# chensh236/ComputerVisionImageStich2

Measured on AMD Instinct MI355X. Metric: warp+blend MPix/s at 4096x4096x3 f32, higher is better.
Workload: dtype f32 (f64 accumulators)

## Files before the change

computervisionimagestich2_amd/capi.py:

```python
import ctypes as C
import os
import re

import numpy as np

_HERE = os.path.dirname(os.path.abspath(__file__))
LIB_PATH = os.environ.get("STITCH_LIB", os.path.join(_HERE, "libstitch_hip.so"))

KERNELS = ("compose", "seam", "mask", "vv_x_fwd", "vv_x_bwd", "vv_y_fwd", "vv_y_bwd", "decimate", "collapse_top", "collapse",
           "collapse_l0", "vv_xbyf", "vv_x_fwd_src", "coarse")
KERNEL_SYMBOLS = {"compose": "k_src_index (source-fused) / k_compose", "seam": "k_seam", "mask": "k_mask", "vv_x_fwd": "k_vv_x_fwd<T, false, false>", "vv_x_bwd": "k_vv_x_bwd",
                  "vv_y_fwd": "k_vv_y_fwd1 / k_vv_y_fwd", "vv_y_bwd": "k_vv_y_bwd_dec", "decimate": "k_decimate", "collapse_top": "k_blend_top",
                  "collapse": "k_collapse<float, false>", "collapse_l0": "k_collapse<T, true>", "vv_xbyf": "k_vv_xbyf<false, float, 0, false>", "vv_x_fwd_src": "k_vv_x_fwd<T, true, false>",
                  "coarse": "k_coarse"}


class StitchError(RuntimeError):
    def __init__(self, code, text):
        super().__init__(f"stitch error {code}: {text}")
        self.code = code


OK, ERR_ARG, ERR_EMPTY_MIDROW, ERR_ZERO_OVERLAP, ERR_PYRAMID, ERR_HIP, ERR_NO_DEVICE = 0, -1, -2, -3, -4, -5, -6

# ... 73 lines not shown
    ("stitch_sift_expn_table", None, vp), ("stitch_sift_elem", None, f64, vp),
)

_lib = None


def lib():
    global _lib
    if _lib is None:
        if not os.path.exists(LIB_PATH):
            raise ImportError(f"{LIB_PATH} is missing: build it with `python -c 'import __graft_entry__ as g; g.build()'` "
                              "(make -C computervisionimagestich2_amd/csrc). There is no CPU fallback.")
        try:
            import torch
        except ImportError:
            pass
        L = C.CDLL(LIB_PATH)
        for name, (res, args) in SIGNATURES.items():
            try:
                f = getattr(L, name)
            except AttributeError:
                raise ImportError(f"{LIB_PATH} does not export {name}: it was built from another include/stitch.h") from None
            f.restype, f.argtypes = res, args
        _lib = L
    return _lib


def _chk(rc):
    if rc < 0:
        raise StitchError(rc, lib().stitch_last_error().decode())
    return rc


def _p(a):
    return a.ctypes.data_as(C.c_void_p)


def _fn(stem, a):
    sfx = {"uint8": "u8", "float32": "f32"}.get(str(a.dtype).rpartition(".")[2])
    if sfx is None:
        raise TypeError(f"unsupported pixel type {a.dtype}")
    return getattr(lib(), stem + sfx)


def _img(a):
    a = np.ascontiguousarray(a)
# ... 596 lines not shown
            assert tuple(out.shape) == (3, self.ch, self.cw) and out.dtype == frame.dtype == mosaic.dtype
            assert frame.dtype == items[0][0].dtype, "one pixel type per batch"
            fn = fn or _fn("stitch_dev_pairs_", frame)
            d.frame, d.fw, d.fh = frame.data_ptr(), frame.shape[2], frame.shape[1]
            d.p = _map8(p)
            d.offx, d.offy = float(offx), float(offy)
            d.mosaic, d.mw, d.mh = mosaic.data_ptr(), mosaic.shape[2], mosaic.shape[1]
            d.ox, d.oy, d.out = int(ox), int(oy), out.data_ptr()
            if out8 is not None:
                import torch
                assert out8.is_cuda and out8.is_contiguous() and out8.dtype == torch.uint8 and tuple(out8.shape) == (3, self.ch, self.cw)
                d.out_u8 = out8.data_ptr()
        _chk(fn(self._h, arr, len(items), _stream()))
        return [it[7] for it in items]

    def status(self, index=0):
        s = Seam()
        _chk(lib().stitch_plan_status_at(self._h, int(index), C.byref(s)))
        return s

    def clear_fault(self):
        _chk(lib().stitch_plan_clear_fault(self._h))

    def set_handoff_spin_limit(self, polls):
        _chk(lib().stitch_plan_set_handoff_spin_limit(self._h, int(polls)))

    def set_profiling_kernel(self, name):
        _chk(lib().stitch_plan_set_profiling_kernel(self._h, KERNELS.index(name)))

    def set_profiling(self, on):
        _chk(lib().stitch_plan_set_profiling(self._h, int(bool(on))))

    def read_profile(self):
        ms, n, l0 = (C.c_double * len(KERNELS))(), (C.c_int * len(KERNELS))(), (C.c_double * len(KERNELS))()
        _chk(lib().stitch_plan_read_profile(self._h, ms, n, l0))
        return {KERNELS[i]: (ms[i], n[i], l0[i]) for i in range(len(KERNELS))}


class Band(_Handle):
    _destroy = "stitch_band_destroy"

    def __init__(self, cw, ch, rank, nranks, split_levels, opts=None):
        self._h = C.c_void_p()
        _chk(lib().stitch_band_create(int(cw), int(ch), int(rank), int(nranks), int(split_levels), C.byref(_opts(opts)), C.byref(self._h)))
        self.cw, self.ch, self.rank, self.nranks, self.split_levels = int(cw), int(ch), int(rank), int(nranks), int(split_levels)
        tot = C.c_int()
# ... 53 lines not shown
```

computervisionimagestich2_amd/csrc/k_fused_sweep.inc:

```
typedef unsigned long long u64;
typedef __attribute__((address_space(1))) u64 gu64;
typedef __attribute__((address_space(1))) unsigned gu32;

struct Wavefront {
    u64* yg;
    int mask_l0;
    unsigned* counter;
    unsigned* abort;
    unsigned* sticky;
    int NR, NC, NP;
    unsigned epoch;
    unsigned spin_limit;
    ZeroTiles zt;
    int ph, y0;
    const double* resume;
    int early_read;
    unsigned long long* dbg;
};

#ifndef STITCH_XBYF_SLEEP
#define STITCH_XBYF_SLEEP 32
#endif
constexpr int WF_GRAN = 7;
__device__ __forceinline__ void granules_publish(u64* base, int lane, unsigned tag, double a, double b, double c, unsigned extra) {
    const u64 w[3] = {(u64)__double_as_longlong(a), (u64)__double_as_longlong(b), (u64)__double_as_longlong(c)};
    __hip_atomic_store((gu64*)(base + 6 * WAVE + lane), ((u64)tag << 32) | extra, __ATOMIC_RELAXED, __HIP_MEMORY_SCOPE_AGENT);
#pragma unroll
    for (int i = 0; i < 3; ++i) {
        __hip_atomic_store((gu64*)(base + (2 * i) * WAVE + lane), ((u64)tag << 32) | (w[i] & 0xffffffffu), __ATOMIC_RELAXED,
                           __HIP_MEMORY_SCOPE_AGENT);
        __hip_atomic_store((gu64*)(base + (2 * i + 1) * WAVE + lane), ((u64)tag << 32) | (w[i] >> 32), __ATOMIC_RELAXED,
                           __HIP_MEMORY_SCOPE_AGENT);
    }
}
__device__ __forceinline__ void granules_issue(const u64* base, int lane, u64 g[WF_GRAN]) {
#pragma unroll
    for (int i = 0; i < WF_GRAN; ++i) g[i] = __hip_atomic_load((gu64*)(base + i * WAVE + lane), __ATOMIC_RELAXED, __HIP_MEMORY_SCOPE_AGENT);
}
__device__ __forceinline__ bool granules_accept(const u64 g[WF_GRAN], unsigned tag, double& a, double& b, double& c, unsigned& extra) {
    bool ok = true;
#pragma unroll
    for (int i = 0; i < WF_GRAN; ++i) ok &= (unsigned)(g[i] >> 32) == tag;
    if (!__all(ok)) return false;
    extra = (unsigned)g[6];
    a = __longlong_as_double((long long)((g[0] & 0xffffffffu) | (g[1] << 32)));
    b = __longlong_as_double((long long)((g[2] & 0xffffffffu) | (g[3] << 32)));
    c = __longlong_as_double((long long)((g[4] & 0xffffffffu) | (g[5] << 32)));
    return true;
}
__device__ __forceinline__ bool granules_consume(const u64* base, int lane, unsigned tag, unsigned* abort, unsigned* sticky,
                                                 unsigned spin_limit, double& a, double& b, double& c, unsigned& extra, bool brisk = false) {
    for (unsigned spins = 0;; ++spins) {
        unsigned seen = 0;
        if (lane == 0)
            seen = (unsigned)(__hip_atomic_load((gu64*)(base + 5 * WAVE + (WAVE - 1)), __ATOMIC_RELAXED, __HIP_MEMORY_SCOPE_AGENT) >> 32);
        seen = __shfl(seen, 0, 64);
        if (seen == tag) {
            u64 g[WF_GRAN];
            bool ok = true;
#pragma unroll
            for (int i = 0; i < WF_GRAN; ++i) {
                g[i] = __hip_atomic_load((gu64*)(base + i * WAVE + lane), __ATOMIC_RELAXED, __HIP_MEMORY_SCOPE_AGENT);
                ok &= (unsigned)(g[i] >> 32) == tag;
            }
            if (__all(ok)) {
                extra = (unsigned)g[6];
                a = __longlong_as_double((long long)((g[0] & 0xffffffffu) | (g[1] << 32)));
                b = __longlong_as_double((long long)((g[2] & 0xffffffffu) | (g[3] << 32)));
                c = __longlong_as_double((long long)((g[4] & 0xffffffffu) | (g[5] << 32)));
                return true;
            }
        }
        {
            if ((spins & 31) == 31) {
                unsigned ab = 0;
                if (lane == 0) ab = __hip_atomic_load((gu32*)abort, __ATOMIC_RELAXED, __HIP_MEMORY_SCOPE_AGENT);
                ab = __shfl(ab, 0, 64);
                if (ab != 0 || spins > spin_limit) {
                    if (lane == 0) {
                        __hip_atomic_store((gu32*)abort, 1u, __ATOMIC_RELAXED, __HIP_MEMORY_SCOPE_AGENT);
                        atomicAdd(sticky, 1u);
                    }
                    return false;
                }
            }
            if (brisk)
                __builtin_amdgcn_s_sleep(2);
            else
                __builtin_amdgcn_s_sleep(STITCH_XBYF_SLEEP);
        }
    }
}

struct Recompute {
    const float* in;
    const double* ckpt;
    const SeamDev* seam;
    ZeroTiles zi;
};
template <bool STAMP, typename PX = float, int MODE = 0, bool BANDED = false>
__global__ __launch_bounds__(64) void k_vv_xbyf(float* __restrict__ data, int w, int h, int pitch, VVK k,
                                                 const double* __restrict__ state_x, long lines, double* __restrict__ state_y,
                                                 Wavefront wf, Recompute rc, typename CollapseSrc<PX, MODE == 2>::type pa) {
    __shared__ __attribute__((aligned(16))) float tile[TS * TP];
    const int lane = threadIdx.x;
    const unsigned nbands = (unsigned)wf.NP * wf.NR;
    unsigned long long seg[8] = {0, 0, 0, 0, 0, 0, 0, 0}, t0 = 0, t1 = 0;
    auto stamp = [&](int i) {
        if (STAMP) {
            t1 = __builtin_amdgcn_s_memtime();
            seg[i] += t1 - t0;
            t0 = t1;
        }
    };
    if (STAMP) t0 = __builtin_amdgcn_s_memtime();
    bool dead = false;
    while (!dead) {
        unsigned q = 0;
        if (lane == 0) q = atomicAdd(wf.counter, 1u);
        q = __builtin_amdgcn_readfirstlane(__shfl(q, 0, 64));
        if (q >= nbands) break;
        const int R = (int)(q / wf.NP), p = (int)(q % wf.NP);
        const int r0 = R * TS, nrows = min(TS, h - r0);
        const int ph = BANDED ? wf.ph : h, y0 = BANDED ? wf.y0 : 0;
// ... 52 lines not shown
#pragma unroll
                for (int i = 0; i < 16; ++i) pre[i] = v;
            } else if (MODE == 1)
                tile_load(in_base, pitch, C * TS, lane, pre);
            else if (gen_frame) {
                if (rc.zi.flags && rc.zi.flags[rc.zi.index(src_pr, R, C)]) {
                    const float o = __uint_as_float(off_outside<PX>());
#pragma unroll
                    for (int i = 0; i < 16; ++i) pre[i] = f4{o, o, o, o};
                } else
                    tile_load(idx_rows, pitch, C * TS, lane, pre);
            }
            if (MODE != 0 && !zero) fetch_ckpt(C);
            return zero;
        };
        auto gather_tile = [&](int C, bool zero) {
            if constexpr (MODE == 2) {
                if (zero || gen_mask) return;
                if (gen_mosaic) mosaic_indices<PX>(ms, C * TS, lane, r0, w, pre);
                src_gather<PX>(rs, pre, pre);
            }
        };
        bool next_zero = false, spec = true;
        if (!const_rows) {
            next_zero = fetch_tile(wf.NC - 1);
            gather_tile(wf.NC - 1, next_zero);
        }
        for (int C = wf.NC - 1; C >= 0; --C) {
            const int c0 = C * TS, ncols = min(TS, w - c0);
            const bool tile_zero = next_zero;
            u64* slot = wf.yg + ((size_t)p * wf.NC + C) * WF_GRAN * WAVE;
            u64 early[WF_GRAN];
            const bool early_on = R > 0 && wf.early_read && (spec || (C & 3) == 0);
            if (early_on) granules_issue(slot, lane, early);
            double f1 = n1, f2 = n2, f3 = n3;
            if (!const_rows) {
                if constexpr (MODE == 2)
                    if (!tile_zero && !gen_mask) src_finish<PX>(gen_frame, pre);
                tile_to_lds(tile, lane, pre);
                if (C > 0) next_zero = fetch_tile(C - 1);
            }
            __syncthreads();
            stamp(1);
            if (MODE != 0 && !const_rows && !tile_zero) {
                float* row = tile + lane * TP;
                if (C == 0) f1 = f2 = f3 = (double)row[0] / k.sumsq;
                const int jfull = ncols & ~15;
                for (int jb = 0; jb < jfull; jb += 16) {
                    float xs[16];
#pragma unroll
                    for (int qq = 0; qq < 4; ++qq) *reinterpret_cast<f4*>(xs + 4 * qq) = *reinterpret_cast<const f4*>(row + jb + 4 * qq);
#pragma unroll
                    for (int u = 0; u < 16; ++u) {
                        double v0 = (double)xs[u];
                        v0 += f1 * k.f1;
                        v0 += f2 * k.f2;
                        v0 += f3 * k.f3;
// ... 51 lines not shown
                        v0 += v3 * k.f3;
                        xs[u] = (float)v0;
                        v3 = v2;
                        v2 = v1;
                        v1 = v0;
                    }
#pragma unroll
                    for (int qq = 0; qq < 4; ++qq) *reinterpret_cast<f4*>(row + jb + 4 * qq) = *reinterpret_cast<const f4*>(xs + 4 * qq);
                }
            }
            __syncthreads();
            stamp(2);
            float* colp = tile + lane;
            double u1, u2, u3;
            unsigned rowbits = 0;
            if (BANDED && R == 0 && wf.resume) {
                const size_t n = (size_t)wf.NP * pitch, i = (size_t)p * pitch + c0 + lane;
                u1 = wf.resume[i], u2 = wf.resume[n + i], u3 = wf.resume[2 * n + i];
                rowbits = __float_as_uint(colp[0]);
            } else if (R == 0) {
                u1 = u2 = u3 = (double)colp[0] / k.sumsq;
                rowbits = __float_as_uint(colp[0]);
            } else {
                const bool hit = early_on && granules_accept(early, (wf.epoch << 12) | (unsigned)R, u1, u2, u3, rowbits);
                if (early_on) spec = hit;
                if (!hit && !granules_consume(slot, lane, (wf.epoch << 12) | (unsigned)R, wf.abort, wf.sticky, wf.spin_limit, u1, u2, u3, rowbits)) {
                    dead = true;
                    break;
                }
            }
            stamp(3);
            const float rowv = __uint_as_float(rowbits);
            const bool y_const = const_rows || (BANDED && pass_row);
            unsigned ynz = 0;
            const double iplus_y = y_const ? (double)rowv : (double)colp[(nrows - 1) * TP];
            const bool y_idle = x_idle && __ballot(lane < ncols && (__double_as_longlong(u1) | __double_as_longlong(u2) |
                                                                   __double_as_longlong(u3)) != 0) == 0;
            for (int j0 = 0; j0 < (y_idle ? 0 : nrows); j0 += 16) {
                if (j0 + 16 <= nrows) {
                    float ys[16];
                    if (y_const) {
#pragma unroll
                        for (int u = 0; u < 16; ++u) ys[u] = rowv;
                    } else {
#pragma unroll
                        for (int u = 0; u < 16; ++u) ys[u] = colp[(j0 + u) * TP];
                    }
#pragma unroll
                    for (int u = 0; u < 16; ++u) {
                        double v0 = (double)ys[u];
                        v0 += u1 * k.f1;
                        v0 += u2 * k.f2;
                        v0 += u3 * k.f3;
                        ys[u] = (float)v0;
                        ynz |= __float_as_uint(ys[u]);
                        u3 = u2;
                        u2 = u1;
                        u1 = v0;
                    }
#pragma unroll
                    for (int u = 0; u < 16; ++u) colp[(j0 + u) * TP] = ys[u];
                } else {
                    for (int j = j0; j < nrows; ++j) {
                        double v0 = y_const ? (double)rowv : (double)colp[j * TP];
                        v0 += u1 * k.f1;
                        v0 += u2 * k.f2;
                        v0 += u3 * k.f3;
                        colp[j * TP] = (float)v0;
                        ynz |= __float_as_uint(colp[j * TP]);
                        u3 = u2;
                        u2 = u1;
                        u1 = v0;
                    }
                }
            }
            if (R < wf.NR - 1)
                granules_publish(slot, lane, (wf.epoch << 12) | (unsigned)(R + 1), u1, u2, u3, pass_row ? rowbits : 0u);
            else {
                const size_t n = (size_t)wf.NP * pitch, i = (size_t)p * pitch + c0 + lane;
                state_y[i] = u1;
                state_y[n + i] = u2;
                state_y[2 * n + i] = u3;
                state_y[3 * n + i] = iplus_y;
            }
            __syncthreads();
            stamp(4);
            bool out_zero = false;
            if (wf.zt.flags) {
                out_zero = __ballot(lane < ncols && ynz != 0) == 0;
                if (lane == 0) wf.zt.flags[wf.zt.index(p, R, C)] = out_zero ? 1 : 0;
            }
            if (!out_zero) tile_store_rows(base, pitch, c0, lane, tile, nrows);
            __syncthreads();
            stamp(5);
        }
    }
    if (STAMP && lane == 0)
        for (int i = 0; i < 8; ++i) wf.dbg[(size_t)blockIdx.x * 8 + i] = seg[i];
}
```

computervisionimagestich2_amd/csrc/k_fused_sweep1.inc:

```
#ifndef STITCH_XY_BUFS
#define STITCH_XY_BUFS 4
#endif
#ifndef STITCH_XY_WGS
#define STITCH_XY_WGS 512
#endif
constexpr int XY_BUFS = STITCH_XY_BUFS, XY_IN = 2, XY_THREADS = 5 * WAVE, XY_MAXNC = 1024, XY_WGS = STITCH_XY_WGS;
struct XYState {
    double u[4][WAVE];
    unsigned extra[WAVE];
};
__global__ __launch_bounds__(XY_THREADS, 3) void k_vv_xby_m(float* __restrict__ data, int w, int h, int pitch, VVK k, const double* __restrict__ state_x,
                                                        long lines, double* __restrict__ state_y, Wavefront wf, const float* __restrict__ zero_page) {
    __shared__ __attribute__((aligned(16))) float tiles[XY_BUFS][TS * TP];
    __shared__ uint8_t s_zf[XY_MAXNC];
    __shared__ XYState st_in[XY_IN], st_out[2];
    __shared__ int c_loaded, c_x, c_y, c_stored, c_in, s_dead;
    __shared__ unsigned s_q;
    const int wave = __builtin_amdgcn_readfirstlane(threadIdx.x >> 6), lane = threadIdx.x & 63;
    const unsigned nbands = (unsigned)wf.NP * wf.NR;
    typedef __attribute__((address_space(3))) int lds_int;
    auto rd = [](int* p) { return __hip_atomic_load((lds_int*)p, __ATOMIC_ACQUIRE, __HIP_MEMORY_SCOPE_WORKGROUP); };
    auto wr = [](int* p, int v) { __hip_atomic_store((lds_int*)p, v, __ATOMIC_RELEASE, __HIP_MEMORY_SCOPE_WORKGROUP); };
    auto wait_ge = [&](int* cnt, int& known, int need) {
        for (unsigned spins = 0; known < need; ++spins) {
// ... 129 lines not shown
                    const int C = NC - 1 - min(j_, NC - 1);
                    const bool z = use_zt && s_zf[C] != 0;
                    tile_load(z ? zero_page : base, z ? 0 : pitch, z ? 0 : C * TS, lane, dst);
                };
                fetch(0, pre[0]);
                fetch(1, pre[1]);
                int stored = 0;
                for (int j0 = 0; j0 < NC; j0 += 2) {
#pragma unroll
                    for (int b = 0; b < 2; ++b) {
                        const int j = j0 + b;
                        if (j < NC) {
                            wait_ge(&c_stored, stored, j - XY_BUFS + 1);
                            tile_to_lds(tiles[j % XY_BUFS], lane, pre[b]);
                            wr(&c_loaded, j + 1);
                            stamp(j);
                        }
                        fetch(j + 2, pre[b]);
                    }
                }
            }
        } else if (wave == 3) {
            int ydone = 0;
            const bool last_band = R == wf.NR - 1;
            for (int j = 0; j < NC; ++j) {
                wait_ge(&c_y, ydone, j + 1);
                const XYState& so = st_out[j & 1];
                const int c0 = (NC - 1 - j) * TS;
                if (!last_band)
                    granules_publish(slot_of(j), lane, tag_out, so.u[0][lane], so.u[1][lane], so.u[2][lane], so.extra[lane]);
                else {
                    const size_t n = (size_t)wf.NP * pitch, i = (size_t)p * pitch + c0 + lane;
                    state_y[i] = so.u[0][lane];
                    state_y[n + i] = so.u[1][lane];
                    state_y[2 * n + i] = so.u[2][lane];
                    state_y[3 * n + i] = so.u[3][lane];
                }
                bool out_zero = false;
                if (use_zt) {
                    if (nrows == TS && c0 + TS <= w) {
                        const float* t = tiles[j % XY_BUFS] + (lane >> 4) * TP + ((lane & 15) << 2);
                        unsigned nz = 0;
#pragma unroll
                        for (int i = 0; i < 16; ++i) {
                            const f4 v = *reinterpret_cast<const f4*>(t + (4 * i) * TP);
                            nz |= __float_as_uint(v.x) | __float_as_uint(v.y) | __float_as_uint(v.z) | __float_as_uint(v.w);
                        }
                        out_zero = __ballot(nz != 0) == 0;
                    }
                    if (lane == 0) wf.zt.flags[wf.zt.index(p, R, NC - 1 - j)] = out_zero ? 1 : 0;
                }
                if (out_zero) {
                } else if (nrows == TS)
                    tile_store(base, pitch, c0, lane, tiles[j % XY_BUFS]);
                else
                    tile_store_rows(base, pitch, c0, lane, tiles[j % XY_BUFS], nrows);
                wr(&c_stored, j + 1);
                stamp(j);
            }
        } else if (R > 0) {
            int ydone = 0;
            u64 g[2][WF_GRAN];
            granules_issue(slot_of(0), lane, g[0]);
            bool alive = true;
            for (int j0 = 0; j0 < NC; j0 += 2) {
#pragma unroll
                for (int b = 0; b < 2; ++b) {
                    const int j = j0 + b;
                    granules_issue(slot_of(min(j + 1, NC - 1)), lane, g[1 - b]);
                    if (j < NC) {
                        double a = 0, bb = 0, c = 0;
                        unsigned extra = 0;
                        if (alive && !granules_accept(g[b], tag_in, a, bb, c, extra)) {
                            alive = granules_consume(slot_of(j), lane, tag_in, wf.abort, wf.sticky, wf.spin_limit, a, bb, c, extra, true);
                            if (!alive) wr(&s_dead, 1);
                        }
                        wait_ge(&c_y, ydone, j - XY_IN + 1);
                        XYState& si = st_in[j % XY_IN];
                        si.u[0][lane] = a, si.u[1][lane] = bb, si.u[2][lane] = c;
                        si.extra[lane] = extra;
                        wr(&c_in, j + 1);
                        stamp(j);
                    }
                }
            }
        }
        __syncthreads();
    }
}
```

computervisionimagestich2_amd/csrc/k_sweeps.inc:

```
constexpr int TS = 64;
constexpr int TP = 68;

__device__ __forceinline__ void tile_load(const float* __restrict__ base, int pitch, int c0, int lane, f4 pre[16]) {
    const float* p = base + (size_t)(lane >> 4) * pitch + c0 + ((lane & 15) << 2);
#pragma unroll
    for (int i = 0; i < 16; ++i) pre[i] = *reinterpret_cast<const f4*>(p + (size_t)(4 * i) * pitch);
}
__device__ __forceinline__ void tile_to_lds(float* tile, int lane, const f4 pre[16]) {
    float* t = tile + (lane >> 4) * TP + ((lane & 15) << 2);
#pragma unroll
    for (int i = 0; i < 16; ++i) *reinterpret_cast<f4*>(t + (4 * i) * TP) = pre[i];
}
__device__ __forceinline__ void tile_store(float* __restrict__ base, int pitch, int c0, int lane, const float* tile) {
    float* p = base + (size_t)(lane >> 4) * pitch + c0 + ((lane & 15) << 2);
    const float* t = tile + (lane >> 4) * TP + ((lane & 15) << 2);
#pragma unroll
    for (int i = 0; i < 16; ++i)
        __builtin_nontemporal_store(*reinterpret_cast<const f4*>(t + (4 * i) * TP), reinterpret_cast<f4*>(p + (size_t)(4 * i) * pitch));
}

struct Bands {
    int nr, h;
};

// ... 541 lines not shown
    const size_t n = (size_t)gridDim.y * pitch, i = ystate_index(blockIdx.y, pitch, x);
    Y2 s;
    if (resume) {
        y2_load(resume, n, i, s);
        stream_rows<false>(p, pitch, h - 1, h, [&](int y, f2 xv) {
            *reinterpret_cast<f2*>(p + (size_t)y * pitch) = y2_step_bwd(s, k, xv);
        });
    } else {
        f2 first;
        y2_triggs(k, state, n, i, s, first);
        *reinterpret_cast<f2*>(p + (size_t)(h - 1) * pitch) = first;
        stream_rows<false>(p, pitch, h - 2, h - 1, [&](int y, f2 xv) {
            *reinterpret_cast<f2*>(p + (size_t)y * pitch) = y2_step_bwd(s, k, xv);
        });
    }
    if (state_out) y2_store(state_out, n, i, s);
}

template <bool ROWZ = false, int NST = YST, bool ZT = true, bool ODD = false, bool XCH = false>
__global__ __launch_bounds__(128) void k_vv_y_bwd_dec(const float* __restrict__ data, int w, int h, int pitch, size_t ps,
                                                      VVK k, const double* __restrict__ state, float* __restrict__ dst,
                                                      int w2, int h2, int dpitch, size_t dps, ZeroTiles zt,
                                                      const double* __restrict__ resume, double* __restrict__ state_out, int wh, int wh2,
                                                      int x_base = 0) {
    static_assert(!(XCH && ODD), "column chunks: even widths");
    __shared__ __attribute__((aligned(16))) float ring[2][YCH][YCOLS];
    const int wave = __builtin_amdgcn_readfirstlane(threadIdx.x >> 6), lane = threadIdx.x & 63;
    const int nchunks = (h + YCH - 1) / YCH;
    constexpr int ADV = ODD ? WAVE - 1 : WAVE;
    const int xl = (blockIdx.x * ADV + lane) * 2, x = XCH ? xl + x_base : xl;
    const bool col_live = x < pitch;
    const int sp = XCH ? (int)gridDim.x * YCOLS : pitch, sx = XCH ? xl : x;
    const float* p = data + blockIdx.y * ps + (col_live ? x : 0);
    Y2 s{};
    f2 first{};
    f2 buf[NST][YCH];
    unsigned long long zm[4] = {0, 0, 0, 0};
    const bool zt_on = ZT && zt.flags != nullptr;
    if (zt_on) {
        const int tA = ((XCH ? x_base : 0) + blockIdx.x * ADV * 2) >> 6, mine = (x >> 6) - tA;
#pragma unroll
        for (int g = 0; g < 4; ++g) {
            if (g * 64 < zt.NR) {
                const int band = g * 64 + lane;
                const bool inb = band < zt.NR;
                const unsigned char fa = inb && tA < zt.NC ? zt.flags[zt.index(blockIdx.y, band, tA)] : 0;
                const unsigned char fb = inb && tA + 1 < zt.NC ? zt.flags[zt.index(blockIdx.y, band, tA + 1)] : 0;
                const unsigned long long mA = __ballot(fa != 0), mB = __ballot(fb != 0);
                unsigned long long m = mine == 0 ? mA : mB;
                if constexpr (ODD) {
                    const unsigned char fc = inb && tA + 2 < zt.NC ? zt.flags[zt.index(blockIdx.y, band, tA + 2)] : 0;
                    const unsigned long long mC = __ballot(fc != 0);
                    m = mine == 2 ? mC : m;
                }
                zm[g] = (x >> 6) < zt.NC ? m : 0ull;
            }
        }
    }
    auto zero_at = [&](int rc) {
        if (!zt_on) return false;
        const int r = rc < h ? rc : h - 1, b = (h - 1 - r) >> 6, g = b >> 6;
        const unsigned long long m = g == 0 ? zm[0] : g == 1 ? zm[1] : g == 2 ? zm[2] : zm[3];
        return ((m >> (b & 63)) & 1) != 0;
    };
    auto chunk_zero = [&](int chunk) { return ROWZ ? false : zero_at(chunk * YCH); };
    const __amdgpu_buffer_rsrc_t rsp = plane_rsrc(data + blockIdx.y * ps, ps);
    const unsigned xo = (col_live ? (unsigned)x : 0u) * 4u, pitch_b = (unsigned)pitch * 4u;
    unsigned next = (unsigned)(h - 1) * pitch_b;
    int issued = 0;
    auto ld = [&](int rc, bool zero) {
        if constexpr (!ZT) {
            const f2 v = ld_row2(rsp, xo, next);
            if (++issued < h) next -= pitch_b;
            return v;
        } else {
            if (ROWZ) zero = zero_at(rc);
            const int r = rc < h ? rc : h - 1, y = h - 1 - r;
            const f2 v = *reinterpret_cast<const f2*>(p + (size_t)(zero ? h - 1 : y) * pitch);
            return zero ? f2{0.f, 0.f} : v;
        }
    };
    if (wave == 0) {
        if (col_live) {
            if (resume)
                y2_load(resume, (size_t)gridDim.y * sp, ystate_index(blockIdx.y, sp, sx), s);
            else
                y2_triggs(k, state, (size_t)gridDim.y * sp, ystate_index(blockIdx.y, sp, sx), s, first);
        }
    }
    if (ZT && zt_on) {
        __shared__ int s_allz;
        bool mine_all = true;
#pragma unroll
        for (int g = 0; g < 4; ++g) {
            if (g * 64 < zt.NR) {
                const int bits = min(64, zt.NR - g * 64);
                const unsigned long long full = bits == 64 ? ~0ull : ((1ull << bits) - 1ull);
                mine_all = mine_all && (zm[g] & full) == full;
            }
        }
        if (wave == 0) {
            const unsigned long long sb = (unsigned long long)__double_as_longlong(s.a1) | (unsigned long long)__double_as_longlong(s.a2) |
                                          (unsigned long long)__double_as_longlong(s.a3) | (unsigned long long)__double_as_longlong(s.b1) |
                                          (unsigned long long)__double_as_longlong(s.b2) | (unsigned long long)__double_as_longlong(s.b3) |
                                          (unsigned long long)(__float_as_uint(first.x) | __float_as_uint(first.y));
            const bool allz0 = __all(mine_all && sb == 0ull);
            if (lane == 0) s_allz = allz0 ? 1 : 0;
        }
        __syncthreads();
        if (s_allz != 0) {
            if (wave == 1) {
                const int tx_ = blockIdx.x * ADV + lane + (XCH ? x_base / 2 : 0);
                if (tx_ < w2 && (!ODD || lane < WAVE - 1)) {
                    float* dc = dst + blockIdx.y * dps + tx_;
                    for (int t = 0; t < h2; ++t) dc[(size_t)t * dpitch] = 0.f;
                }
            } else if (state_out && col_live)
                y2_store(state_out, (size_t)gridDim.y * sp, ystate_index(blockIdx.y, sp, sx), s);
            return;
        }
    }
    if (wave == 0) {
#pragma unroll
        for (int st = 0; st < NST - 1; ++st) {
            const bool z = chunk_zero(st);
#pragma unroll
            for (int u = 0; u < YCH; ++u) buf[st][u] = ld(st * YCH + u, z);
        }
    }
// ... 106 lines not shown
```

computervisionimagestich2_amd/csrc/stitch_hip.hip:

```cpp
#include <hip/hip_runtime.h>

#include <cmath>
#include <cstdarg>
#include <cstdio>
#include <cstdlib>
#include <algorithm>
#include <cstring>
#include <atomic>
#include <condition_variable>
#include <functional>
#include <list>
#include <mutex>
#include <string>
#include <thread>
#include <vector>

#include "stitch.h"
#include "stitch_kernels.hpp"

#pragma clang fp contract(off)

using namespace sk;

namespace {

thread_local std::string g_err;


int fail(int code, const char* fmt, ...) {
    char buf[512];
    va_list ap;
    va_start(ap, fmt);
    vsnprintf(buf, sizeof buf, fmt, ap);
    va_end(ap);
    g_err = buf;
    return code;
}

#define HIPCHK(expr)                                                                                              \
    do {                                                                                                          \
// ... 360 lines not shown
                StageTimer t(p, s, src && l == 0 ? STITCH_K_VV_X_FWD_SRC : STITCH_K_VV_X_FWD, l);
                if (src && l == 0) {
                    if (rcmp)
                        k_vv_x_fwd<PX, true, true><<<nb, 64, 0, s>>>(a.g, p->T, a.w, a.pitch, lines, p->vvk, p->state, mk, pa, zt, zi, p->ckpt, bd);
                    else
                        k_vv_x_fwd<PX, true><<<nb, 64, 0, s>>>(a.g, p->T, a.w, a.pitch, lines, p->vvk, p->state, mk, pa, zt, zi, nullptr, bd);
                } else if (rcmp)
                    k_vv_x_fwd<PX, false, true><<<nb, 64, 0, s>>>(a.g, p->T, a.w, a.pitch, lines, p->vvk, p->state, mk, NoPairArgs{}, zt, ZeroTiles{}, p->ckpt, bd);
                else
                    k_vv_x_fwd<PX, false><<<nb, 64, 0, s>>>(a.g, p->T, a.w, a.pitch, lines, p->vvk, p->state, mk, NoPairArgs{}, zt, ZeroTiles{}, nullptr, bd);
            }
            Wavefront wf{};
            wf.yg = p->wf_yg;
            wf.counter = p->wf_ctrl + (size_t)l * 16;
            wf.abort = p->wf_ctrl + WF_CTRL_WORDS - 16;
            wf.sticky = p->wf_ctrl + WF_CTRL_WORDS;
            wf.spin_limit = p->wf_spin_limit;
            wf.NR = NR;
            wf.NC = (a.w + TS - 1) / TS;
            wf.NP = np;
            const size_t gran_words = (size_t)wf.NP * wf.NC * WF_GRAN * WAVE;
            k_clear_words<<<(int)std::min<size_t>((gran_words + 255) / 256, 2048), 256, 0, s>>>(p->wf_yg, gran_words);
            wf.epoch = 1;
            wf.mask_l0 = mk.enabled;
            wf.zt = zt;
            wf.early_read = p->wf_early_read;
            const long ntiles = (long)wf.NP * wf.NR;
            double* state_y = p->state + 4 * (size_t)p->cap * 7 * (a.h + 64);
            {
                StageTimer t(p, s, STITCH_K_VV_XBYF, l);
                const int wg = (int)std::min<long>(ntiles, p->wf_max_wgs);
                Recompute rcv{};
                if (rcmp) {
                    rcv.in = a.g;
                    rcv.ckpt = p->ckpt;
                    rcv.seam = p->d_seam;
                    if (src && l == 0) rcv.zi = zi;
                }
                if (p->wf_dbg && l == 0) {
                    wf.dbg = p->wf_dbg;
                    k_vv_xbyf<true><<<wg, 64, 0, s>>>(p->T, a.w, a.h, a.pitch, p->vvk, p->state, lines, state_y, wf, rcv, NoPairArgs{});
                } else if (rcmp && src && l == 0)
                    k_vv_xbyf<false, PX, 2><<<wg, 64, 0, s>>>(p->T, a.w, a.h, a.pitch, p->vvk, p->state, lines, state_y, wf, rcv, pa);
                else if (rcmp)
                    k_vv_xbyf<false, float, 1><<<wg, 64, 0, s>>>(p->T, a.w, a.h, a.pitch, p->vvk, p->state, lines, state_y, wf, rcv, NoPairArgs{});
                else
                    k_vv_xbyf<false><<<wg, 64, 0, s>>>(p->T, a.w, a.h, a.pitch, p->vvk, p->state, lines, state_y, wf, rcv, NoPairArgs{});
            }
            StageTimer t(p, s, STITCH_K_VV_Y_BWD, l);
            dim3 g((a.pitch + YCOLS - 1) / YCOLS, np);
            if ((a.w & 1) == 0 && !p->no_fuse) {
                if (rowz)
                    k_vv_y_bwd_dec<true><<<g, 128, 0, s>>>(p->T, a.w, a.h, a.pitch, a.ps, p->vvk, state_y, b.g, b.w, b.h, b.pitch, b.ps, zt, nullptr, nullptr, a.h, b.h);
                else
                    k_vv_y_bwd_dec<false><<<g, 128, 0, s>>>(p->T, a.w, a.h, a.pitch, a.ps, p->vvk, state_y, b.g, b.w, b.h, b.pitch, b.ps, zt, nullptr, nullptr, a.h, b.h);
                decimated = true;
            } else if (odd_dec) {
                const dim3 go((b.w + WAVE - 2) / (WAVE - 1), np);
                if (rowz)
                    k_vv_y_bwd_dec<true, YST, true, true><<<go, 128, 0, s>>>(p->T, a.w, a.h, a.pitch, a.ps, p->vvk, state_y, b.g, b.w, b.h, b.pitch, b.ps, zt, nullptr, nullptr, a.h, b.h);
                else
                    k_vv_y_bwd_dec<false, YST, true, true><<<go, 128, 0, s>>>(p->T, a.w, a.h, a.pitch, a.ps, p->vvk, state_y, b.g, b.w, b.h, b.pitch, b.ps, zt, nullptr, nullptr, a.h, b.h);
                decimated = true;
            } else
                k_vv_y_bwd<<<g, 64, 0, s>>>(p->T, a.h, a.pitch, a.ps, p->vvk, state_y, nullptr, nullptr);
        } else if (p->opts.blur_kind == 0) {
            const bool mover = p->tune.mover != 0;
            const bool src0 = src && l == 0;
            const bool xby = do_x && do_y && lone_fused_level(p, n, l);
            const double* ystate = p->state;
            if (do_x && mover && !zt.flags && (nbx <= 340 || (src0 && nbx <= 1024))) {
                {
                    StageTimer t(p, s, src0 ? STITCH_K_VV_X_FWD_SRC : STITCH_K_VV_X_FWD, l);
                    if (src0)
                        k_vv_x_m<true, PX, true><<<nbx, 192, 0, s>>>(a.g, p->T, a.w, a.pitch, lines, p->vvk, p->state, mk, bd, pa);
                    else
                        k_vv_x_m<true><<<nbx, 192, 0, s>>>(a.g, p->T, a.w, a.pitch, lines, p->vvk, p->state, mk, bd, NoPairArgs{});
                }
                StageTimer t(p, s, STITCH_K_VV_X_BWD, l);
                if (xby) {
                } else if (nbx <= 340)
                    k_vv_x_m<false><<<nbx, 192, 0, s>>>(p->T, p->T, a.w, a.pitch, lines, p->vvk, p->state, mk, bd, NoPairArgs{});
                else
                    k_vv_x_bwd<<<nbx, 64, 0, s>>>(p->T, a.w, a.pitch, lines, p->vvk, p->state, mk, bd);
            } else if (do_x) {
// ... 1347 lines not shown
        HIPCHK(hipStreamSynchronize(p->last_stream));
        p->pending = false;
    }
    if (p->h_wf_abort && *p->h_wf_abort != p->wf_abort_seen)
        return fail(STITCH_ERR_HIP,
                    "fused sweep: %u hand-off wait(s) timed out in this or an earlier queued call on the plan (every result since the "
                    "last stitch_plan_clear_fault is invalid)",
                    *p->h_wf_abort - p->wf_abort_seen);
    const SeamDev& sd = p->h_seam[index];
    seam_to_public(sd, seam_out);
    if (sd.status == -2) return fail(STITCH_ERR_EMPTY_MIDROW, "blend: channel 0 of a's middle row is empty (pair %d)", index);
    if (sd.status == -3) return fail(STITCH_ERR_ZERO_OVERLAP, "blend: a and b do not overlap on the middle row (pair %d)", index);
    return STITCH_OK;
}

int stitch_plan_status(stitch_plan* p, stitch_seam* seam_out) { return stitch_plan_status_at(p, 0, seam_out); }

int stitch_plan_set_handoff_spin_limit(stitch_plan* p, unsigned polls) {
    if (!p) return fail(STITCH_ERR_ARG, "null plan");
    p->wf_spin_limit = polls;
    return STITCH_OK;
}

int stitch_plan_clear_fault(stitch_plan* p) {
    if (!p) return fail(STITCH_ERR_ARG, "null plan");
    if (p->pending) {
        HIPCHK(hipStreamSynchronize(p->last_stream));
        p->pending = false;
    }
    if (p->h_wf_abort) p->wf_abort_seen = *p->h_wf_abort;
    return STITCH_OK;
}

int stitch_plan_capacity(const stitch_plan* p) { return p ? p->cap : 0; }
int stitch_plan_coarse_from(const stitch_plan* p) { return p ? p->coarse_from : 0; }
int stitch_plan_fast_paths(const stitch_plan* p) {
    if (!p) return 0;
    int f = 0;
    if (p->mask_opt) f |= STITCH_FAST_IMPLICIT_MASK;
    if (p->src_fuse) f |= STITCH_FAST_SOURCE_FUSED;
    if (p->wf_levels > 0) f |= STITCH_FAST_FUSED_SWEEP;
    if (p->wf_levels > 0 && p->zero_tiles && !p->no_fuse && ((p->lv[0].w & 1) == 0 || (p->lv[0].w >= 3 && p->tune.odd_dec != 0)) &&
        (p->lv[0].h + TS - 1) / TS <= 256 && !(p->tune.gate64 && (p->lv[0].h % TS || (p->lv[0].w & 1))))
        f |= STITCH_FAST_ZERO_TILES;
    if (!p->no_fuse && p->opts.blur_kind == 0 && !p->blur_skip && p->L >= 2 && ((p->lv[0].w & 1) == 0 || (p->lv[0].w >= 3 && p->tune.odd_dec != 0)) && p->lv[0].h > 1)
        f |= STITCH_FAST_FUSED_DECIMATE;
// ... 482 lines not shown
```

Before: 24520.

## Pack wavefront hand-off granules into 48-bit payloads with zero-tile shortcut

Repacks the per-lane hand-off state (three doubles plus row bits) from seven 32-bit-tagged words into four or five words with 16-bit tags and 48-bit payloads. An all-zero wave now publishes a single zero-flag word that consumers accept immediately. The row word is skipped when it is not needed, and the courier loop is specialised on that case. It also adds constant-fill row detection for masked level 0, an occupancy hint on k_vv_xbyf, and device counters exposed through a new API. The aims are less global-memory atomic traffic and shorter polling latency, at the cost of tag width, more complex packing, and extra atomics for the counters.

```diff
diff --git a/computervisionimagestich2_amd/capi.py b/computervisionimagestich2_amd/capi.py
--- a/computervisionimagestich2_amd/capi.py
+++ b/computervisionimagestich2_amd/capi.py
@@ -119,6 +119,7 @@
             except AttributeError:
                 raise ImportError(f"{LIB_PATH} does not export {name}: it was built from another include/stitch.h") from None
             f.restype, f.argtypes = res, args
+        L.stitch_plan_handoff_counts.restype, L.stitch_plan_handoff_counts.argtypes = i32, [vp, vp]
         _lib = L
     return _lib
 
@@ -761,6 +762,11 @@
     def clear_fault(self):
         _chk(lib().stitch_plan_clear_fault(self._h))
 
+    def handoff_counts(self):
+        out = (C.c_uint64 * 3)()
+        _chk(lib().stitch_plan_handoff_counts(self._h, out))
+        return tuple(int(v) for v in out)
+
     def set_handoff_spin_limit(self, polls):
         _chk(lib().stitch_plan_set_handoff_spin_limit(self._h, int(polls)))
 
diff --git a/computervisionimagestich2_amd/csrc/k_fused_sweep.inc b/computervisionimagestich2_amd/csrc/k_fused_sweep.inc
--- a/computervisionimagestich2_amd/csrc/k_fused_sweep.inc
+++ b/computervisionimagestich2_amd/csrc/k_fused_sweep.inc
@@ -21,55 +21,63 @@
 #ifndef STITCH_XBYF_SLEEP
 #define STITCH_XBYF_SLEEP 32
 #endif
-constexpr int WF_GRAN = 7;
-__device__ __forceinline__ void granules_publish(u64* base, int lane, unsigned tag, double a, double b, double c, unsigned extra) {
-    const u64 w[3] = {(u64)__double_as_longlong(a), (u64)__double_as_longlong(b), (u64)__double_as_longlong(c)};
-    __hip_atomic_store((gu64*)(base + 6 * WAVE + lane), ((u64)tag << 32) | extra, __ATOMIC_RELAXED, __HIP_MEMORY_SCOPE_AGENT);
-#pragma unroll
-    for (int i = 0; i < 3; ++i) {
-        __hip_atomic_store((gu64*)(base + (2 * i) * WAVE + lane), ((u64)tag << 32) | (w[i] & 0xffffffffu), __ATOMIC_RELAXED,
-                           __HIP_MEMORY_SCOPE_AGENT);
-        __hip_atomic_store((gu64*)(base + (2 * i + 1) * WAVE + lane), ((u64)tag << 32) | (w[i] >> 32), __ATOMIC_RELAXED,
-                           __HIP_MEMORY_SCOPE_AGENT);
+constexpr int WF_GRAN = 5;
+constexpr int WF_POLL = 3;
+constexpr unsigned WF_ZERO = 0x8000u;
+constexpr u64 WF_PAYLOAD = (1ull << 48) - 1;
+__device__ __forceinline__ bool granules_publish(u64* base, int lane, int live, unsigned tag, double a, double b, double c, unsigned extra, bool row) {
+    const u64 wa = (u64)__double_as_longlong(a), wb = (u64)__double_as_longlong(b), wc = (u64)__double_as_longlong(c), t = (u64)tag << 48;
+    if (__ballot(lane < live && ((wa | wb | wc) != 0 || (row && extra != 0))) == 0) {
+        if (lane == WAVE - 1)
+            __hip_atomic_store((gu64*)(base + WF_POLL * WAVE + lane), (u64)(tag | WF_ZERO) << 48, __ATOMIC_RELAXED, __HIP_MEMORY_SCOPE_AGENT);
+        return true;
     }
+    if (row) __hip_atomic_store((gu64*)(base + 4 * WAVE + lane), t | extra, __ATOMIC_RELAXED, __HIP_MEMORY_SCOPE_AGENT);
+    __hip_atomic_store((gu64*)(base + lane), t | (wa & WF_PAYLOAD), __ATOMIC_RELAXED, __HIP_MEMORY_SCOPE_AGENT);
+    __hip_atomic_store((gu64*)(base + WAVE + lane), t | (wa >> 48) | ((wb & 0xffffffffull) << 16), __ATOMIC_RELAXED, __HIP_MEMORY_SCOPE_AGENT);
+    __hip_atomic_store((gu64*)(base + 2 * WAVE + lane), t | (wb >> 32) | ((wc & 0xffffull) << 32), __ATOMIC_RELAXED, __HIP_MEMORY_SCOPE_AGENT);
+    __hip_atomic_store((gu64*)(base + 3 * WAVE + lane), t | (wc >> 16), __ATOMIC_RELAXED, __HIP_MEMORY_SCOPE_AGENT);
+    return false;
 }
-__device__ __forceinline__ void granules_issue(const u64* base, int lane, u64 g[WF_GRAN]) {
-#pragma unroll
-    for (int i = 0; i < WF_GRAN; ++i) g[i] = __hip_atomic_load((gu64*)(base + i * WAVE + lane), __ATOMIC_RELAXED, __HIP_MEMORY_SCOPE_AGENT);
+__device__ __forceinline__ void granules_issue(const u64* base, int lane, u64 g[WF_GRAN], bool row) {
+#pragma unroll
+    for (int i = 0; i < 4; ++i) g[i] = __hip_atomic_load((gu64*)(base + i * WAVE + lane), __ATOMIC_RELAXED, __HIP_MEMORY_SCOPE_AGENT);
+    g[4] = 0;
+    if (row) g[4] = __hip_atomic_load((gu64*)(base + 4 * WAVE + lane), __ATOMIC_RELAXED, __HIP_MEMORY_SCOPE_AGENT);
 }
-__device__ __forceinline__ bool granules_accept(const u64 g[WF_GRAN], unsigned tag, double& a, double& b, double& c, unsigned& extra) {
-    bool ok = true;
-#pragma unroll
-    for (int i = 0; i < WF_GRAN; ++i) ok &= (unsigned)(g[i] >> 32) == tag;
+__device__ __forceinline__ bool granules_accept(const u64 g[WF_GRAN], unsigned tag, double& a, double& b, double& c, unsigned& extra, bool row) {
+    const unsigned polled = (unsigned)__builtin_amdgcn_readlane((int)(g[WF_POLL] >> 48), WAVE - 1);
+    if (polled == (tag | WF_ZERO)) {
+        a = b = c = 0.0;
+        extra = 0;
+        return true;
+    }
+    bool ok = !row || (unsigned)(g[4] >> 48) == tag;
+#pragma unroll
+    for (int i = 0; i < 4; ++i) ok &= (unsigned)(g[i] >> 48) == tag;
     if (!__all(ok)) return false;
-    extra = (unsigned)g[6];
-    a = __longlong_as_double((long long)((g[0] & 0xffffffffu) | (g[1] << 32)));
-    b = __longlong_as_double((long long)((g[2] & 0xffffffffu) | (g[3] << 32)));
-    c = __longlong_as_double((long long)((g[4] & 0xffffffffu) | (g[5] << 32)));
+    extra = (unsigned)g[4];
+    a = __longlong_as_double((long long)((g[0] & WF_PAYLOAD) | (g[1] << 48)));
+    b = __longlong_as_double((long long)(((g[1] & WF_PAYLOAD) >> 16) | (g[2] << 32)));
+    c = __longlong_as_double((long long)(((g[2] & WF_PAYLOAD) >> 32) | (g[3] << 16)));
     return true;
 }
 __device__ __forceinline__ bool granules_consume(const u64* base, int lane, unsigned tag, unsigned* abort, unsigned* sticky,
-                                                 unsigned spin_limit, double& a, double& b, double& c, unsigned& extra, bool brisk = false) {
+                                                 unsigned spin_limit, double& a, double& b, double& c, unsigned& extra, bool row, bool brisk = false) {
     for (unsigned spins = 0;; ++spins) {
         unsigned seen = 0;
         if (lane == 0)
-            seen = (unsigned)(__hip_atomic_load((gu64*)(base + 5 * WAVE + (WAVE - 1)), __ATOMIC_RELAXED, __HIP_MEMORY_SCOPE_AGENT) >> 32);
+            seen = (unsigned)(__hip_atomic_load((gu64*)(base + WF_POLL * WAVE + (WAVE - 1)), __ATOMIC_RELAXED, __HIP_MEMORY_SCOPE_AGENT) >> 48);
         seen = __shfl(seen, 0, 64);
+        if (seen == (tag | WF_ZERO)) {
+            a = b = c = 0.0;
+            extra = 0;
+            return true;
+        }
         if (seen == tag) {
             u64 g[WF_GRAN];
-            bool ok = true;
-#pragma unroll
-            for (int i = 0; i < WF_GRAN; ++i) {
-                g[i] = __hip_atomic_load((gu64*)(base + i * WAVE + lane), __ATOMIC_RELAXED, __HIP_MEMORY_SCOPE_AGENT);
-                ok &= (unsigned)(g[i] >> 32) == tag;
-            }
-            if (__all(ok)) {
-                extra = (unsigned)g[6];
-                a = __longlong_as_double((long long)((g[0] & 0xffffffffu) | (g[1] << 32)));
-                b = __longlong_as_double((long long)((g[2] & 0xffffffffu) | (g[3] << 32)));
-                c = __longlong_as_double((long long)((g[4] & 0xffffffffu) | (g[5] << 32)));
-                return true;
-            }
+            granules_issue(base, lane, g, row);
+            if (granules_accept(g, tag, a, b, c, extra, row)) return true;
         }
         {
             if ((spins & 31) == 31) {
@@ -99,7 +107,7 @@
     ZeroTiles zi;
 };
 template <bool STAMP, typename PX = float, int MODE = 0, bool BANDED = false>
-__global__ __launch_bounds__(64) void k_vv_xbyf(float* __restrict__ data, int w, int h, int pitch, VVK k,
+__global__ __launch_bounds__(64, (MODE == 0 && !STAMP) ? 3 : 2) void k_vv_xbyf(float* __restrict__ data, int w, int h, int pitch, VVK k,
                                                  const double* __restrict__ state_x, long lines, double* __restrict__ state_y,
                                                  Wavefront wf, Recompute rc, typename CollapseSrc<PX, MODE == 2>::type pa) {
     __shared__ __attribute__((aligned(16))) float tile[TS * TP];
@@ -198,6 +206,9 @@
             }
         };
         bool next_zero = false, spec = true;
+        unsigned sent = 0;
+        const bool fill_rows = !BANDED && const_rows && wf.mask_l0 == 2;
+        unsigned recorded = 0;
         if (!const_rows) {
             next_zero = fetch_tile(wf.NC - 1);
             gather_tile(wf.NC - 1, next_zero);
@@ -208,7 +219,7 @@
             u64* slot = wf.yg + ((size_t)p * wf.NC + C) * WF_GRAN * WAVE;
             u64 early[WF_GRAN];
             const bool early_on = R > 0 && wf.early_read && (spec || (C & 3) == 0);
-            if (early_on) granules_issue(slot, lane, early);
+            if (early_on) granules_issue(slot, lane, early, pass_row);
             double f1 = n1, f2 = n2, f3 = n3;
             if (!const_rows) {
                 if constexpr (MODE == 2)
@@ -306,15 +317,24 @@
                 u1 = u2 = u3 = (double)colp[0] / k.sumsq;
                 rowbits = __float_as_uint(colp[0]);
             } else {
-                const bool hit = early_on && granules_accept(early, (wf.epoch << 12) | (unsigned)R, u1, u2, u3, rowbits);
+                const bool hit = early_on && granules_accept(early, (wf.epoch << 12) | (unsigned)R, u1, u2, u3, rowbits, pass_row);
                 if (early_on) spec = hit;
-                if (!hit && !granules_consume(slot, lane, (wf.epoch << 12) | (unsigned)R, wf.abort, wf.sticky, wf.spin_limit, u1, u2, u3, rowbits)) {
+                if (!hit && !granules_consume(slot, lane, (wf.epoch << 12) | (unsigned)R, wf.abort, wf.sticky, wf.spin_limit, u1, u2, u3, rowbits, pass_row)) {
                     dead = true;
                     break;
                 }
             }
             stamp(3);
             const float rowv = __uint_as_float(rowbits);
+            unsigned fillbits = 0;
+            if (fill_rows) {
+                const double u = (double)rowv / k.sumsq;
+                double v0 = (double)rowv;
+                v0 += u * k.f1;
+                v0 += u * k.f2;
+                v0 += u * k.f3;
+                fillbits = __float_as_uint((float)v0);
+            }
             const bool y_const = const_rows || (BANDED && pass_row);
             unsigned ynz = 0;
             const double iplus_y = y_const ? (double)rowv : (double)colp[(nrows - 1) * TP];
@@ -337,7 +357,7 @@
                         v0 += u2 * k.f2;
                         v0 += u3 * k.f3;
                         ys[u] = (float)v0;
-                        ynz |= __float_as_uint(ys[u]);
+                        ynz |= __float_as_uint(ys[u]) ^ fillbits;
                         u3 = u2;
                         u2 = u1;
                         u1 = v0;
@@ -351,7 +371,7 @@
                         v0 += u2 * k.f2;
                         v0 += u3 * k.f3;
                         colp[j * TP] = (float)v0;
-                        ynz |= __float_as_uint(colp[j * TP]);
+                        ynz |= __float_as_uint(colp[j * TP]) ^ fillbits;
                         u3 = u2;
                         u2 = u1;
                         u1 = v0;
@@ -359,7 +379,7 @@
                 }
             }
             if (R < wf.NR - 1)
-                granules_publish(slot, lane, (wf.epoch << 12) | (unsigned)(R + 1), u1, u2, u3, pass_row ? rowbits : 0u);
+                sent += granules_publish(slot, lane, ncols, (wf.epoch << 12) | (unsigned)(R + 1), u1, u2, u3, rowbits, pass_row) ? 0x10000u : 1u;
             else {
                 const size_t n = (size_t)wf.NP * pitch, i = (size_t)p * pitch + c0 + lane;
                 state_y[i] = u1;
@@ -372,12 +392,19 @@
             bool out_zero = false;
             if (wf.zt.flags) {
                 out_zero = __ballot(lane < ncols && ynz != 0) == 0;
+                if (!BANDED && pass_row && R == 0 && wf.mask_l0 == 2) out_zero = false;
                 if (lane == 0) wf.zt.flags[wf.zt.index(p, R, C)] = out_zero ? 1 : 0;
+                if (fill_rows && out_zero) ++recorded;
             }
             if (!out_zero) tile_store_rows(base, pitch, c0, lane, tile, nrows);
             __syncthreads();
             stamp(5);
         }
+        if (lane == 0 && sent != 0) {
+            atomicAdd((u64*)(wf.sticky + 2), (u64)(sent & 0xffffu));
+            atomicAdd((u64*)(wf.sticky + 4), (u64)(sent >> 16));
+        }
+        if (lane == 0 && recorded != 0) atomicAdd((u64*)(wf.sticky + 6), (u64)recorded);
     }
     if (STAMP && lane == 0)
         for (int i = 0; i < 8; ++i) wf.dbg[(size_t)blockIdx.x * 8 + i] = seg[i];
diff --git a/computervisionimagestich2_amd/csrc/k_fused_sweep1.inc b/computervisionimagestich2_amd/csrc/k_fused_sweep1.inc
--- a/computervisionimagestich2_amd/csrc/k_fused_sweep1.inc
+++ b/computervisionimagestich2_amd/csrc/k_fused_sweep1.inc
@@ -175,13 +175,14 @@
             }
         } else if (wave == 3) {
             int ydone = 0;
+            unsigned sent = 0;
             const bool last_band = R == wf.NR - 1;
             for (int j = 0; j < NC; ++j) {
                 wait_ge(&c_y, ydone, j + 1);
                 const XYState& so = st_out[j & 1];
                 const int c0 = (NC - 1 - j) * TS;
                 if (!last_band)
-                    granules_publish(slot_of(j), lane, tag_out, so.u[0][lane], so.u[1][lane], so.u[2][lane], so.extra[lane]);
+                    sent += granules_publish(slot_of(j), lane, min(TS, w - c0), tag_out, so.u[0][lane], so.u[1][lane], so.u[2][lane], so.extra[lane], pass_row) ? 0x10000u : 1u;
                 else {
                     const size_t n = (size_t)wf.NP * pitch, i = (size_t)p * pitch + c0 + lane;
                     state_y[i] = so.u[0][lane];
@@ -211,32 +212,43 @@
                 wr(&c_stored, j + 1);
                 stamp(j);
             }
+            if (lane == 0 && sent != 0) {
+                atomicAdd((u64*)(wf.sticky + 2), (u64)(sent & 0xffffu));
+                atomicAdd((u64*)(wf.sticky + 4), (u64)(sent >> 16));
+            }
         } else if (R > 0) {
-            int ydone = 0;
-            u64 g[2][WF_GRAN];
-            granules_issue(slot_of(0), lane, g[0]);
-            bool alive = true;
-            for (int j0 = 0; j0 < NC; j0 += 2) {
-#pragma unroll
-                for (int b = 0; b < 2; ++b) {
-                    const int j = j0 + b;
-                    granules_issue(slot_of(min(j + 1, NC - 1)), lane, g[1 - b]);
-                    if (j < NC) {
-                        double a = 0, bb = 0, c = 0;
-                        unsigned extra = 0;
-                        if (alive && !granules_accept(g[b], tag_in, a, bb, c, extra)) {
-                            alive = granules_consume(slot_of(j), lane, tag_in, wf.abort, wf.sticky, wf.spin_limit, a, bb, c, extra, true);
-                            if (!alive) wr(&s_dead, 1);
-                        }
-                        wait_ge(&c_y, ydone, j - XY_IN + 1);
-                        XYState& si = st_in[j % XY_IN];
-                        si.u[0][lane] = a, si.u[1][lane] = bb, si.u[2][lane] = c;
-                        si.extra[lane] = extra;
-                        wr(&c_in, j + 1);
-                        stamp(j);
-                    }
-                }
-            }
+            auto courier = [&](auto ROW) {
+                constexpr bool row = decltype(ROW)::value;
+                int ydone = 0;
+                u64 g[2][WF_GRAN];
+                granules_issue(slot_of(0), lane, g[0], row);
+                bool alive = true;
+                for (int j0 = 0; j0 < NC; j0 += 2) {
+#pragma unroll
+                    for (int b = 0; b < 2; ++b) {
+                        const int j = j0 + b;
+                        granules_issue(slot_of(min(j + 1, NC - 1)), lane, g[1 - b], row);
+                        if (j < NC) {
+                            double a = 0, bb = 0, c = 0;
+                            unsigned extra = 0;
+                            if (alive && !granules_accept(g[b], tag_in, a, bb, c, extra, row)) {
+                                alive = granules_consume(slot_of(j), lane, tag_in, wf.abort, wf.sticky, wf.spin_limit, a, bb, c, extra, row, true);
+                                if (!alive) wr(&s_dead, 1);
+                            }
+                            wait_ge(&c_y, ydone, j - XY_IN + 1);
+                            XYState& si = st_in[j % XY_IN];
+                            si.u[0][lane] = a, si.u[1][lane] = bb, si.u[2][lane] = c;
+                            si.extra[lane] = extra;
+                            wr(&c_in, j + 1);
+                            stamp(j);
+                        }
+                    }
+                }
+            };
+            if (pass_row)
+                courier(std::true_type{});
+            else
+                courier(std::false_type{});
         }
         __syncthreads();
     }
diff --git a/computervisionimagestich2_amd/csrc/k_sweeps.inc b/computervisionimagestich2_amd/csrc/k_sweeps.inc
--- a/computervisionimagestich2_amd/csrc/k_sweeps.inc
+++ b/computervisionimagestich2_amd/csrc/k_sweeps.inc
@@ -587,7 +587,7 @@
                                                       VVK k, const double* __restrict__ state, float* __restrict__ dst,
                                                       int w2, int h2, int dpitch, size_t dps, ZeroTiles zt,
                                                       const double* __restrict__ resume, double* __restrict__ state_out, int wh, int wh2,
-                                                      int x_base = 0) {
+                                                      int x_base = 0, int fill_l0 = 0) {
     static_assert(!(XCH && ODD), "column chunks: even widths");
     __shared__ __attribute__((aligned(16))) float ring[2][YCH][YCOLS];
     const int wave = __builtin_amdgcn_readfirstlane(threadIdx.x >> 6), lane = threadIdx.x & 63;
@@ -629,6 +629,8 @@
         return ((m >> (b & 63)) & 1) != 0;
     };
     auto chunk_zero = [&](int chunk) { return ROWZ ? false : zero_at(chunk * YCH); };
+    const bool fill_on = ZT && zt_on && fill_l0 != 0 && blockIdx.y % 7 == 6;
+    const int dummy = fill_on ? 0 : h - 1;
     const __amdgpu_buffer_rsrc_t rsp = plane_rsrc(data + blockIdx.y * ps, ps);
     const unsigned xo = (col_live ? (unsigned)x : 0u) * 4u, pitch_b = (unsigned)pitch * 4u;
     unsigned next = (unsigned)(h - 1) * pitch_b;
@@ -641,8 +643,9 @@
         } else {
             if (ROWZ) zero = zero_at(rc);
             const int r = rc < h ? rc : h - 1, y = h - 1 - r;
-            const f2 v = *reinterpret_cast<const f2*>(p + (size_t)(zero ? h - 1 : y) * pitch);
-            return zero ? f2{0.f, 0.f} : v;
+            const f2 v = *reinterpret_cast<const f2*>(p + (size_t)(zero ? dummy : y) * pitch);
+            const unsigned keep = (zero && !fill_on) ? 0u : ~0u;
+            return f2{__uint_as_float(__float_as_uint(v.x) & keep), __uint_as_float(__float_as_uint(v.y) & keep)};
         }
     };
     if (wave == 0) {
@@ -669,7 +672,7 @@
                                           (unsigned long long)__double_as_longlong(s.a3) | (unsigned long long)__double_as_longlong(s.b1) |
                                           (unsigned long long)__double_as_longlong(s.b2) | (unsigned long long)__double_as_longlong(s.b3) |
                                           (unsigned long long)(__float_as_uint(first.x) | __float_as_uint(first.y));
-            const bool allz0 = __all(mine_all && sb == 0ull);
+            const bool allz0 = __all(mine_all && sb == 0ull) && !fill_on;
             if (lane == 0) s_allz = allz0 ? 1 : 0;
         }
         __syncthreads();
diff --git a/computervisionimagestich2_amd/csrc/stitch_hip.hip b/computervisionimagestich2_amd/csrc/stitch_hip.hip
--- a/computervisionimagestich2_amd/csrc/stitch_hip.hip
+++ b/computervisionimagestich2_amd/csrc/stitch_hip.hip
@@ -16,6 +16,7 @@
 #include <vector>
 
 #include "stitch.h"
+#include "stitch_handoff.h"
 #include "stitch_kernels.hpp"
 
 #pragma clang fp contract(off)
@@ -422,7 +423,7 @@
             const size_t gran_words = (size_t)wf.NP * wf.NC * WF_GRAN * WAVE;
             k_clear_words<<<(int)std::min<size_t>((gran_words + 255) / 256, 2048), 256, 0, s>>>(p->wf_yg, gran_words);
             wf.epoch = 1;
-            wf.mask_l0 = mk.enabled;
+            wf.mask_l0 = mk.enabled ? (zt.flags ? 2 : 1) : 0;
             wf.zt = zt;
             wf.early_read = p->wf_early_read;
             const long ntiles = (long)wf.NP * wf.NR;
@@ -449,18 +450,19 @@
             }
             StageTimer t(p, s, STITCH_K_VV_Y_BWD, l);
             dim3 g((a.pitch + YCOLS - 1) / YCOLS, np);
+            const int fill_l0 = wf.mask_l0 == 2;
             if ((a.w & 1) == 0 && !p->no_fuse) {
                 if (rowz)
-                    k_vv_y_bwd_dec<true><<<g, 128, 0, s>>>(p->T, a.w, a.h, a.pitch, a.ps, p->vvk, state_y, b.g, b.w, b.h, b.pitch, b.ps, zt, nullptr, nullptr, a.h, b.h);
+                    k_vv_y_bwd_dec<true><<<g, 128, 0, s>>>(p->T, a.w, a.h, a.pitch, a.ps, p->vvk, state_y, b.g, b.w, b.h, b.pitch, b.ps, zt, nullptr, nullptr, a.h, b.h, 0, fill_l0);
                 else
-                    k_vv_y_bwd_dec<false><<<g, 128, 0, s>>>(p->T, a.w, a.h, a.pitch, a.ps, p->vvk, state_y, b.g, b.w, b.h, b.pitch, b.ps, zt, nullptr, nullptr, a.h, b.h);
+                    k_vv_y_bwd_dec<false><<<g, 128, 0, s>>>(p->T, a.w, a.h, a.pitch, a.ps, p->vvk, state_y, b.g, b.w, b.h, b.pitch, b.ps, zt, nullptr, nullptr, a.h, b.h, 0, fill_l0);
                 decimated = true;
             } else if (odd_dec) {
                 const dim3 go((b.w + WAVE - 2) / (WAVE - 1), np);
                 if (rowz)
-                    k_vv_y_bwd_dec<true, YST, true, true><<<go, 128, 0, s>>>(p->T, a.w, a.h, a.pitch, a.ps, p->vvk, state_y, b.g, b.w, b.h, b.pitch, b.ps, zt, nullptr, nullptr, a.h, b.h);
+                    k_vv_y_bwd_dec<true, YST, true, true><<<go, 128, 0, s>>>(p->T, a.w, a.h, a.pitch, a.ps, p->vvk, state_y, b.g, b.w, b.h, b.pitch, b.ps, zt, nullptr, nullptr, a.h, b.h, 0, fill_l0);
                 else
-                    k_vv_y_bwd_dec<false, YST, true, true><<<go, 128, 0, s>>>(p->T, a.w, a.h, a.pitch, a.ps, p->vvk, state_y, b.g, b.w, b.h, b.pitch, b.ps, zt, nullptr, nullptr, a.h, b.h);
+                    k_vv_y_bwd_dec<false, YST, true, true><<<go, 128, 0, s>>>(p->T, a.w, a.h, a.pitch, a.ps, p->vvk, state_y, b.g, b.w, b.h, b.pitch, b.ps, zt, nullptr, nullptr, a.h, b.h, 0, fill_l0);
                 decimated = true;
             } else
                 k_vv_y_bwd<<<g, 64, 0, s>>>(p->T, a.h, a.pitch, a.ps, p->vvk, state_y, nullptr, nullptr);
@@ -1854,6 +1856,17 @@
     return STITCH_OK;
 }
 
+int stitch_plan_handoff_counts(stitch_plan* p, uint64_t out[3]) {
+    if (!p || !out) return fail(STITCH_ERR_ARG, "null plan or output");
+    if (p->pending) {
+        HIPCHK(hipStreamSynchronize(p->last_stream));
+        p->pending = false;
+    }
+    out[0] = out[1] = out[2] = 0;
+    if (p->wf_ctrl) HIPCHK(hipMemcpy(out, p->wf_ctrl + WF_CTRL_WORDS + 2, 3 * sizeof(uint64_t), hipMemcpyDeviceToHost));
+    return STITCH_OK;
+}
+
 int stitch_plan_clear_fault(stitch_plan* p) {
     if (!p) return fail(STITCH_ERR_ARG, "null plan");
     if (p->pending) {
diff --git a/include/stitch_handoff.h b/include/stitch_handoff.h
--- /dev/null
+++ b/include/stitch_handoff.h
@@ -0,0 +1,14 @@
+#ifndef STITCH_HANDOFF_H
+#define STITCH_HANDOFF_H
+#include <stdint.h>
+
+#include "stitch.h"
+
+#ifdef __cplusplus
+extern "C" {
+#endif
+int stitch_plan_handoff_counts(stitch_plan *plan, uint64_t out[3]);
+#ifdef __cplusplus
+}
+#endif
+#endif
```

New measurement: 24930 (median of 6 runs). 1.02x the previous value.
